# bearcove/loona

Measured on AMD Instinct MI355X. Metric: Huffman header-literal decode GiB/s (device-resident) at 1/2/4/8 MI355X, higher is better.
Workload: dtype u8

## Files before the change

### loona_amd/csrc/hpk_ctx.hip

```cpp
#include <stdio.h>
#include <string.h>
#include <sys/mman.h>

#include <initializer_list>

#include "hpk_device.h"

#define HPK_VERSION "hpk 0.39 gfx950 decode v39 (every batch: wave fills, each wave with its own LDS window and image, lookups in a 13-bit two-symbol table, longest-first queue, slot end offsets by DPP, nontemporal window loads stopping at the chunk's last byte, nontemporal write-back; chunks by guided self-scheduling from 4M literals, fixed 96-literal chunks below; fills and long-literal phase: body steps with no fit tests while >= 31 bits are left (29 with the 12-bit table), then the wave fills' tails as four masked lookups with no fit test per code (checked steps only for a 14..30-bit code or a cut code in the tail) and the other kernels' checked tails (the long phase's at its refill points); long literals one lane each streaming from HBM after the fills, dense ranges listed longest-first; literals of >= 8 KiB by a whole workgroup in speculative pieces; compacted-output form: wave fills packed per workgroup from an LDS cursor into a bound layout made from the input offsets, each lane storing its two literals in unaligned 16-byte pieces; small-call mode: a persistent kernel behind a host-mapped doorbell); encode v5 (byte-balanced workgroup ranges, start map and DPP segmented scan, run accumulator, LDS image, live chunks only)"

static thread_local std::string t_last_error;

int hpk_set_err(const char* what, hipError_t e) {
    char buf[256];
    snprintf(buf, sizeof buf, "%s: %s", what, hipGetErrorString(e));
    t_last_error = buf;
    return HPK_E_DEVICE;
}

int hpk_set_err_msg(const char* what, int code) {
    t_last_error = what;
    return code;
}


extern "C" const char* hpk_version(void) { return HPK_VERSION; }

extern "C" const char* hpk_last_error(const hpk_ctx*) { return t_last_error.c_str(); }

extern "C" hpk_ctx* hpk_ctx_create(int device) {
    const hpk_tables* t = hpk_get_tables();
    if (!t) { hpk_set_err_msg("code table build failed", HPK_E_INVAL); return nullptr; }
    int ndev = 0;
    hipError_t e = hipGetDeviceCount(&ndev);
    if (e != hipSuccess || ndev <= 0) { hpk_set_err("hipGetDeviceCount", e); return nullptr; }
    if (device < 0 || device >= ndev) { hpk_set_err_msg("device index out of range", HPK_E_INVAL); return nullptr; }
    hpk_ctx* c = new hpk_ctx();
    c->device = device;
    auto fail = [&](const char* what, hipError_t err) {
        hpk_set_err(what, err);
        hpk_ctx_destroy(c);
        return (hpk_ctx*)nullptr;
    };
    if ((e = hipSetDevice(device)) != hipSuccess) return fail("hipSetDevice", e);
    hipDeviceProp_t prop;
    if ((e = hipGetDeviceProperties(&prop, device)) != hipSuccess) return fail("hipGetDeviceProperties", e);
    if (strncmp(prop.gcnArchName, "gfx950", 6) != 0) {
        hpk_set_err_msg("libhpk kernels are built for gfx950 only", HPK_E_NODEVICE);
        delete c;
        return nullptr;
    }
    c->num_cu = prop.multiProcessorCount;
    if ((e = hipStreamCreateWithFlags(&c->own, hipStreamNonBlocking)) != hipSuccess) return fail("hipStreamCreate", e);
    c->stream = c->own;
    if ((e = hipMalloc(&c->d_lut2, sizeof(t->lut2))) != hipSuccess) return fail("hipMalloc lut2", e);
    if ((e = hipMemcpy(c->d_lut2, t->lut2, sizeof(t->lut2), hipMemcpyHostToDevice)) != hipSuccess)
        return fail("upload lut2", e);
    if ((e = hipMalloc(&c->d_lut3, sizeof(t->lut3))) != hipSuccess) return fail("hipMalloc lut3", e);
    if ((e = hipMemcpy(c->d_lut3, t->lut3, sizeof(t->lut3), hipMemcpyHostToDevice)) != hipSuccess)
        return fail("upload lut3", e);
    if ((e = hipMalloc(&c->d_lut13, sizeof(t->lut13))) != hipSuccess) return fail("hipMalloc lut13", e);
    if ((e = hipMemcpy(c->d_lut13, t->lut13, sizeof(t->lut13), hipMemcpyHostToDevice)) != hipSuccess)
        return fail("upload lut13", e);
    if ((e = hipMalloc(&c->d_lo, sizeof(t->lo))) != hipSuccess) return fail("hipMalloc lo", e);
    if ((e = hipMalloc(&c->d_codes, 2 * 257 * sizeof(uint32_t))) != hipSuccess) return fail("hipMalloc codes", e);
    uint32_t packed[2 * 257];
    for (int s = 0; s < 257; ++s) {
        packed[s] = t->code[s];
        packed[257 + s] = t->len[s];
    }
    if ((e = hipMemcpy(c->d_lo, t->lo, sizeof(t->lo), hipMemcpyHostToDevice)) != hipSuccess) return fail("upload lo", e);
    if ((e = hipMemcpy(c->d_codes, packed, sizeof(packed), hipMemcpyHostToDevice)) != hipSuccess) return fail("upload codes", e);
    if ((e = hipHostMalloc((void**)&c->h_err, 64, hipHostMallocMapped | hipHostMallocCoherent)) != hipSuccess)
        return fail("hipHostMalloc err flag", e);
    *c->h_err = 0;
    if ((e = hipHostGetDevicePointer((void**)&c->d_err, c->h_err, 0)) != hipSuccess) return fail("err flag pointer", e);
    return c;
}

static int grow(void** p, size_t* cap, size_t need) {
    if (need <= *cap) return HPK_E_OK;
    size_t n = need + need / 4 + 4096;
    (void)hipFree(*p);
    *p = nullptr;
    *cap = 0;
    HIP_TRY(hipMalloc(p, n));
    *cap = n;
    return HPK_E_OK;
}

static int slot_acquire(hpk_ctx* c, hpk_slot** slot) {
    hpk_slot* s = nullptr;
    bool any = false;
    for (hpk_slot& k : c->slots) {
        if (k.used && k.stream == c->stream) s = &k;
        any |= k.used;
    }
    if (!s) {
        if (any && !c->slot_events) {
            c->slot_events = true;
            HIP_TRY(hipStreamSynchronize(c->own));
            for (hpk_slot& k : c->slots)
                if (k.stream == c->own) k.ev_set = false;
        }
        int j = 0;
        while (j < hpk_ctx::kSlots && c->slots[j].used) ++j;
        if (j == hpk_ctx::kSlots) {
            j = c->slot_next;
            c->slot_next = (j + 1) % hpk_ctx::kSlots;
            if (c->slots[j].ev_set) HIP_TRY(hipEventSynchronize(c->slots[j].ev));
        }
        s = &c->slots[j];
        s->stream = c->stream;
    }
    if (c->slot_events && !s->ev) HIP_TRY(hipEventCreateWithFlags(&s->ev, hipEventDisableTiming));
    *slot = s;
    return HPK_E_OK;
}

struct slot_need {
    DevBuf* buf;
    size_t bytes;
};
static int slot_reserve(hpk_ctx* c, hpk_slot* s, std::initializer_list<slot_need> needs) {
    bool small = false;
    for (const slot_need& nd : needs) small |= nd.buf->cap < nd.bytes;
    if (small) {
        if (s->ev_set)
            HIP_TRY(hipEventSynchronize(s->ev));
        else if (s->used)
            HIP_TRY(hipStreamSynchronize(c->own));
        for (const slot_need& nd : needs)
            if (int rc = grow(&nd.buf->p, &nd.buf->cap, nd.bytes)) return rc;
    }
    s->used = true;
    return HPK_E_OK;
}

static int slot_commit(hpk_ctx* c, hpk_slot* s) {
    if (!c->slot_events && c->stream == c->own) return HPK_E_OK;
    if (!s->ev) HIP_TRY(hipEventCreateWithFlags(&s->ev, hipEventDisableTiming));
    HIP_TRY(hipEventRecord(s->ev, c->stream));
    s->ev_set = true;
    return HPK_E_OK;
}

extern "C" void hpk_ctx_destroy(hpk_ctx* c) {
    if (!c) return;
    (void)hipSetDevice(c->device);
    (void)hpk_persist_stop(c);
    if (c->sm_stream) (void)hipStreamDestroy(c->sm_stream);
    if (c->h_sm) (void)hipHostFree(c->h_sm);
    (void)hipFree(c->d_sm_dev);
    (void)hipStreamSynchronize(c->stream);
    (void)hipFree(c->d_lut2);
    (void)hipFree(c->d_lut3);
    (void)hipFree(c->d_lut13);
    (void)hipFree(c->d_lo);
    (void)hipFree(c->d_codes);
    (void)hipFree(c->d_in);
    (void)hipFree(c->d_out);
    (void)hipFree(c->d_meta);
    (void)hipFree(c->d_st);
    if (c->h_err) (void)hipHostFree(c->h_err);
    if (c->h_pin) (void)hipHostFree(c->h_pin);
    for (hpk_slot& s : c->slots) {
        if (s.ev_set) (void)hipEventSynchronize(s.ev);
        for (DevBuf* b : {&s.long_list, &s.cp_bound, &s.cp_tmp, &s.cp_cursor, &s.pk_scratch, &s.pk_bound, &s.pk_tmp})
            (void)hipFree(b->p);
        if (s.ev) (void)hipEventDestroy(s.ev);
    }
    for (int j = 0; j < hpk_ctx::kMaxChunks; ++j) {
        if (c->ev_in[j]) (void)hipEventDestroy(c->ev_in[j]);
        if (c->ev_run[j]) (void)hipEventDestroy(c->ev_run[j]);
        if (c->ev_out[j]) (void)hipEventDestroy(c->ev_out[j]);
    }
    if (c->h2d) (void)hipStreamDestroy(c->h2d);
    if (c->d2h) (void)hipStreamDestroy(c->d2h);
    if (c->own) (void)hipStreamDestroy(c->own);
    delete c;
}

extern "C" int hpk_ctx_set_stream(hpk_ctx* c, void* s) {
    if (!c) return HPK_E_INVAL;
    if (s == HPK_STREAM_LEGACY)
        c->stream = (hipStream_t)0;
    else
        c->stream = s ? (hipStream_t)s : c->own;
    return HPK_E_OK;
}

extern "C" int hpk_host_register(void* ptr, size_t bytes) {
    if (!ptr || !bytes) return hpk_set_err_msg("null range", HPK_E_INVAL);
    HIP_TRY(hipHostRegister(ptr, bytes, hipHostRegisterDefault));
    return HPK_E_OK;
}

extern "C" int hpk_host_unregister(void* ptr) {
    if (!ptr) return hpk_set_err_msg("null pointer", HPK_E_INVAL);
    HIP_TRY(hipHostUnregister(ptr));
    return HPK_E_OK;
}

int hpk_ctx_pinned(hpk_ctx* c, size_t bytes, void** p) {
    if (bytes > c->h_pin_cap) {
        HIP_TRY(hipSetDevice(c->device));
        HIP_TRY(hipStreamSynchronize(c->stream));
        if (c->d2h) HIP_TRY(hipStreamSynchronize(c->d2h));
        if (c->h_pin) (void)hipHostFree(c->h_pin);
        c->h_pin = nullptr;
        c->h_pin_cap = 0;
        const size_t cap = bytes + bytes / 4 + (1u << 20);
        HIP_TRY(hipHostMalloc(&c->h_pin, cap, hipHostMallocDefault));
        c->h_pin_cap = cap;
    }
    *p = c->h_pin;
    return HPK_E_OK;
}

extern "C" int hpk_ctx_set_decode_kernel(hpk_ctx* c, int kind) {
    if (!c || kind < HPK_DECODE_AUTO || kind > HPK_DECODE_WAVE) return hpk_set_err_msg("bad decode kernel", HPK_E_INVAL);
    c->decode_kernel = kind;
    return HPK_E_OK;
}

extern "C" void* hpk_ctx_stream(hpk_ctx* c) { return c ? (void*)c->stream : nullptr; }

extern "C" int hpk_ctx_set_small_mode(hpk_ctx* c, uint32_t max_literals, int workgroups, uint32_t idle_ms) {
    if (!c) return HPK_E_INVAL;
    HIP_TRY(hipSetDevice(c->device));
    if (max_literals == 0) {
        const int rc = hpk_persist_stop(c);
        c->sm_max = 0;
        return rc;
    }
    if (workgroups < 1 || workgroups > 16 || workgroups >= c->num_cu || idle_ms < 1 || idle_ms > 10000 ||
        max_literals > (uint32_t)workgroups * 256u * 64u)
        return hpk_set_err_msg("small mode: 1-16 workgroups, 1-10000 ms idle, at most 64 literals per lane", HPK_E_INVAL);
    if (!c->h_sm) {
        HIP_TRY(hipStreamCreateWithFlags(&c->sm_stream, hipStreamNonBlocking));
        HIP_TRY(hipHostMalloc(&c->h_sm, 256, hipHostMallocMapped | hipHostMallocCoherent));
        memset(c->h_sm, 0, 256);
        HIP_TRY(hipHostGetDevicePointer(&c->d_sm, c->h_sm, 0));
        HIP_TRY(hipMalloc(&c->d_sm_dev, 128));
    }
    if (c->sm_launched && (workgroups != c->sm_wgs || idle_ms != c->sm_idle_ms))
        if (int rc = hpk_persist_stop(c)) return rc;
    c->sm_max = max_literals;
    c->sm_wgs = workgroups;
    c->sm_idle_ms = idle_ms;
    return c->sm_launched ? HPK_E_OK : hpk_persist_start(c);
}

extern "C" int hpk_ctx_sync(hpk_ctx* c) {
    if (!c) return HPK_E_INVAL;
    HIP_TRY(hipStreamSynchronize(c->stream));
    return HPK_E_OK;
}

static int check_offsets(const uint32_t* off, uint32_t n, size_t cap) {
    for (uint32_t i = 0; i < n; ++i)
        if (off[i + 1] < off[i]) return hpk_set_err_msg("offsets must be non-decreasing", HPK_E_INVAL);
    if (off[n] > cap || off[n] > HPK_MAX_OFFSET) return hpk_set_err_msg("offsets pass the blob's capacity", HPK_E_INVAL);
    return HPK_E_OK;
}

static int take_err(hpk_ctx* c) {
    if (!__atomic_exchange_n(c->h_err, 0u, __ATOMIC_ACQ_REL)) return HPK_E_OK;
    return hpk_set_err_msg("a batch had non-monotone offsets or offsets past a blob's capacity (HPK_BAD_OFFSETS)",
                           HPK_E_INVAL);
}

extern "C" int hpk_ctx_check(hpk_ctx* c) {
    if (!c) return HPK_E_INVAL;
    HIP_TRY(hipStreamSynchronize(c->stream));
    return take_err(c);
}

static int call_end(hpk_ctx* c, int flags) {
    if (flags & HPK_ASYNC) return HPK_E_OK;
    HIP_TRY(hipStreamSynchronize(c->stream));
    return take_err(c);
}

typedef int (*launch_fn)(hpk_ctx*, const hpk_batch&);

static int decode_region(hpk_ctx* c, const hpk_batch& b) {
    hpk_slot* s;
    int rc;
    if ((rc = slot_acquire(c, &s)) || (rc = slot_reserve(c, s, {{&s->long_list, 4 * (size_t)b.n}}))) return rc;
    if ((rc = hpk_launch_decode(c, b, s->long_list.as<uint32_t>()))) return rc;
    return slot_commit(c, s);
}

static uint32_t clamp_cap(size_t cap) { return cap > HPK_MAX_OFFSET ? HPK_MAX_OFFSET : (uint32_t)cap; }

static int queue_chunks(launch_fn fn, hpk_ctx* c, const uint8_t* in_blob, const uint32_t* in_off, uint8_t* out_blob,
                        const uint32_t* out_off, uint32_t* out_len, uint8_t* status, uint32_t n, size_t in_bytes,
                        size_t out_bytes, int chunks, const uint32_t* cut, uint32_t* d_in_off, uint32_t* d_out_off,
                        uint32_t* d_len);

static int host_begin(launch_fn fn, hpk_ctx* c, const uint8_t* in_blob, size_t in_cap, const uint32_t* in_off,
                      uint32_t n, uint8_t* out_blob, size_t out_cap, const uint32_t* out_off, uint32_t* out_len,
                      uint8_t* status, bool trusted, int* nchunks, uint32_t* cut) {
    *nchunks = 0;
    if (!trusted && (check_offsets(in_off, n, in_cap) || check_offsets(out_off, n, out_cap))) return HPK_E_INVAL;
    if (n == 0) return HPK_E_OK;
    const size_t in_bytes = in_off[n], out_bytes = out_off[n];
    if ((in_bytes && !in_blob) || (out_bytes && !out_blob)) return hpk_set_err_msg("null blob", HPK_E_INVAL);
    int rc;
    if ((rc = grow((void**)&c->d_in, &c->d_in_cap, in_bytes + 16))) return rc;
    if ((rc = grow((void**)&c->d_out, &c->d_out_cap, out_bytes + 16))) return rc;
// ... 285 lines not shown
```

### loona_amd/csrc/hpk_wave.h

```cpp
#pragma once
#include <type_traits>

#include "hpk_decode_kernel.h"
#include "hpk_huge.h"
#include "hpk_long.h"

#ifndef HPK_BODY_UNROLL
#define HPK_BODY_UNROLL 4
#endif
#ifndef HPK_WAVE_TAB
#define HPK_WAVE_TAB 4
#endif
#ifndef HPK_CW_LANE_DIAG
#define HPK_CW_LANE_DIAG 0
#endif
#ifndef HPK_NT_STORE
#define HPK_NT_STORE 1
#endif
#ifndef HPK_NT_LOAD
#define HPK_NT_LOAD 1
#endif
#ifndef HPK_TAIL_MASKED
#define HPK_TAIL_MASKED 1
#endif
#ifndef HPK_WIN_CUT
#define HPK_WIN_CUT 1
#endif

namespace hpkdec {

typedef uint32_t v4u32 __attribute__((ext_vector_type(4)));
__device__ __forceinline__ void st16(uint4* p, const uint4 v) {
    if (HPK_NT_STORE) {
        const v4u32 x = {v.x, v.y, v.z, v.w};
        __builtin_nontemporal_store(x, reinterpret_cast<v4u32*>(p));
    } else {
        *p = v;
    }
}
__device__ __forceinline__ uint4 ld16(const uint4* p) {
    if (HPK_NT_LOAD) {
        const v4u32 x = __builtin_nontemporal_load(reinterpret_cast<const v4u32*>(p));
        return make_uint4(x.x, x.y, x.z, x.w);
    }
    return *p;
}

template <int kWinB, int kImgB, int kTab>
struct GeoW {
    static constexpr int kWaves = 16, kBlock = kWaves * 64;
    static constexpr int kWaveBytes = kWinB + kImgB;
    static constexpr int kLutBytes = 4 << lut_bits<kTab>();
    static constexpr int kLutOff = kLoBytes;
    static constexpr int kDummyOff = kLutOff + kLutBytes;
    static constexpr int kWaveOff = kDummyOff + 256;
    static constexpr int kCtrOff = kWaveOff + kWaves * kWaveBytes;
    static constexpr int kLdsBytes = kCtrOff + 64 + (int)kHugeMax * 4;
    static constexpr int kImg = kImgB;
    static_assert(kLoBytes % 16 == 0, "16-byte aligned carve-outs");
    static constexpr int kWinRounds = (kWinB / 16 + 63) / 64;
    static constexpr int kFlushRounds = (kImg / 16 + 1 + 63) / 64;
    static_assert(kLdsBytes <= 163840, "LDS budget (160 KiB per CU on gfx950)");
    static_assert(kWinB % 16 == 0 && kImgB % 16 == 0 && kWinB < 65536 && kImgB < 131072, "entry packing");
    static_assert(kWaves * kWaveBytes >= huge_lds_bytes<kBlock>(), "huge-phase LDS");
};

__device__ __forceinline__ uint32_t wave_incl_scan(uint32_t x, uint32_t lane) {
    x += (uint32_t)__builtin_amdgcn_update_dpp(0, (int)x, 0x111, 0xF, 0xF, false);
    x += (uint32_t)__builtin_amdgcn_update_dpp(0, (int)x, 0x112, 0xF, 0xF, false);
    x += (uint32_t)__builtin_amdgcn_update_dpp(0, (int)x, 0x114, 0xF, 0xF, false);
    x += (uint32_t)__builtin_amdgcn_update_dpp(0, (int)x, 0x118, 0xF, 0xF, false);
    const uint32_t r0 = (uint32_t)__builtin_amdgcn_readlane((int)x, 15);
    const uint32_t r1 = (uint32_t)__builtin_amdgcn_readlane((int)x, 31);
    const uint32_t r2 = (uint32_t)__builtin_amdgcn_readlane((int)x, 47);
    return x + (lane >= 16u ? r0 : 0u) + (lane >= 32u ? r1 : 0u) + (lane >= 48u ? r2 : 0u);
}

template <int kMode, int kWinB, int kImgB, uint32_t kChunk, int kGuided, int kRank, bool kCompact = false>
__global__ __launch_bounds__(1024) void hpk_decode_wave(DecodeArgs a) {
    constexpr int kTab = HPK_WAVE_TAB;
    using G = GeoW<kWinB, kMode == 3 ? kImgB - 64 : kImgB, kTab>;
    constexpr int kStore = kMode == 2 ? kNoStore : kPred;
    constexpr uint32_t kStamps = 13;
    __shared__ uint32_t s_dg[kMode == 3 ? G::kWaves * kStamps : 1];
    uint32_t tq = kMode == 3 ? (uint32_t)__builtin_amdgcn_s_memtime() : 0u;
    const uint32_t t_start = tq;
    auto dg_add = [&](int i, uint32_t v) {
        if (kMode == 3 && (threadIdx.x & 63u) == 0u) atomicAdd(&s_dg[(threadIdx.x >> 6) * kStamps + i], v);
    };
    auto stamp = [&](int i) {
        if (kMode == 3) {
            const uint32_t t = (uint32_t)__builtin_amdgcn_s_memtime();
            dg_add(i, t - tq);
            tq = t;
        }
    };
    constexpr int R = G::kWinRounds, F = G::kFlushRounds;
    __shared__ __attribute__((aligned(16))) uint8_t smem[G::kLdsBytes];
    uint16_t* s_lo = reinterpret_cast<uint16_t*>(smem);
    uint32_t* s_lut = reinterpret_cast<uint32_t*>(smem + G::kLutOff);
    uint32_t* s_ctr = reinterpret_cast<uint32_t*>(smem + G::kCtrOff);
    uint32_t* s_huge = s_ctr + 16;
    const uint32_t tid = threadIdx.x, lane = tid & 63u, wv = tid >> 6;
    const uint32_t BA = (uint32_t)((uint64_t)a.n * blockIdx.x / gridDim.x);
    const uint32_t BB = (uint32_t)((uint64_t)a.n * (blockIdx.x + 1) / gridDim.x);
    static_assert(G::kBlock == 1024, "the dense check's two offsets rounds");
    const uint32_t c0 = kGuided == 2 ? kChunk : max(kChunk, (BB - BA) / 32u);
    const uint32_t cur0 = kGuided == 0 ? BA + (uint32_t)((uint64_t)(BB - BA) * wv / G::kWaves) : min(BA + wv * c0, BB);
    const uint32_t ce0 =
        kGuided == 0 ? BA + (uint32_t)((uint64_t)(BB - BA) * (wv + 1) / G::kWaves) : min(cur0 + c0, BB);
    const uint32_t gin0 = a.in_off[cur0];
    const uint32_t gend0 = HPK_WIN_CUT ? a.in_off[ce0] : 0u;
    const uint32_t gout0 = kCompact ? 0u : a.out_off[cur0];
    const uint32_t kd = min(BB - BA, 2048u);
    uint32_t dv0[2], dv1[2];
#pragma unroll
    for (int r = 0; r < 2; ++r) {
        const uint32_t tt = BA + min(tid + (uint32_t)G::kBlock * r, kd ? kd - 1u : 0u);
        dv0[r] = a.in_off[tt];
        dv1[r] = a.in_off[tt + 1u];
    }
    for (uint32_t t = tid; t < kLoBytes / 16; t += G::kBlock)
        reinterpret_cast<uint4*>(s_lo)[t] = reinterpret_cast<const uint4*>(a.lo)[t];
    for (uint32_t t = tid; t < (uint32_t)G::kLutBytes / 16; t += G::kBlock)
        reinterpret_cast<uint4*>(s_lut)[t] = reinterpret_cast<const uint4*>(kTab == 4 ? a.lut13 : kTab == 3 ? a.lut3 : a.lut2)[t];
    if (tid < 16) s_ctr[tid] = tid == 7 && kGuided ? min(G::kWaves * c0, BB - BA) : 0u;
    if (kMode == 3)
        for (uint32_t t = tid; t < (uint32_t)G::kWaves * kStamps; t += G::kBlock) s_dg[t] = 0;
    const uint32_t in_end = min(a.in_off[a.n], a.in_cap) + a.in_mis;
    const uint32_t last16 = in_end ? (in_end - 1) >> 4 : 0;
    const uint32_t in0 = kCompact ? a.in_off[0] : 0u;
    auto ulay = [&](uint32_t i, uint32_t io) -> uint32_t {
        const uint32_t d = io - in0, q = __umulhi(d, 0xCCCCCCCDu) >> 2;
        return d + 3u * q + (((d - 5u * q) * 39u) >> 6) + 4u * i;
    };
    auto oof = [&](uint32_t i) -> uint32_t { return kCompact ? ulay(i, a.in_off[i]) : a.out_off[i]; };
    if (kCompact && blockIdx.x == 0 && tid == 0) a.co_off[a.n] = ulay(a.n, a.in_off[a.n]);
    const uint32_t wg0 = kCompact && BA < BB ? oof(BA) : 0u;
    auto leave = [&](uint32_t i, uint32_t nb) {
        if (kCompact) a.co_off[i] = wg0 + atomicAdd(&s_ctr[9], ((nb * 8u) / 5u + 3u) & ~3u);
        if (nb >= HPK_HUGE_MIN && nb < kHugeLimit) {
            const uint32_t h = atomicAdd(&s_ctr[8], 1u);
            if (h < kHugeMax) {
                s_huge[h] = i;
                return;
            }
        }
        if (nb >= a.long_big)
            a.long_list[BA + atomicAdd(&s_ctr[1], 1u)] = i;
        else
            a.long_list[BB - 1u - atomicAdd(&s_ctr[2], 1u)] = i;
    };
    __syncthreads();
    bool dense = false;
    {
        uint32_t dlb = 0, dtb = 0;
#pragma unroll
        for (int r = 0; r < 2; ++r) {
            if (tid + (uint32_t)G::kBlock * r < kd) {
                const uint32_t nb = min(dv1[r] - dv0[r], 1u << 20);
                dtb += nb;
                dlb += nb >= a.long_min ? nb : 0u;
            }
        }
#pragma unroll
        for (int d = 32; d >= 1; d >>= 1) {
            dlb += __shfl_xor(dlb, d);
            dtb += __shfl_xor(dtb, d);
        }
        if (lane == 0 && dtb) {
            atomicAdd(&s_ctr[4], dlb);
            atomicAdd(&s_ctr[5], dtb);
        }
        __syncthreads();
        if (s_ctr[4] > s_ctr[5] / 2u) {
            uint32_t* const s_cls = reinterpret_cast<uint32_t*>(smem + G::kWaveOff);
            if (tid < 64) s_cls[tid] = 0;
            __syncthreads();
            bool no = false;
            for (uint32_t i = BA + tid; i < BB; i += G::kBlock) {
                const uint32_t p0 = a.in_off[i], p1 = a.in_off[i + 1];
                const uint32_t q0 = kCompact ? ulay(i, p0) : a.out_off[i], q1 = kCompact ? ulay(i + 1u, p1) : a.out_off[i + 1];
                const bool ok = p0 <= p1 && p1 <= a.in_cap && q0 <= q1 && q1 <= a.out_cap &&
                                (uint64_t)(q1 - q0) >= (uint64_t)(p1 - p0) * 8u / 5u;
                if (!ok) {
                    no = true;
                    continue;
                }
                const uint32_t nb = p1 - p0;
                if (!(nb >= HPK_HUGE_MIN && nb < kHugeLimit)) atomicAdd(&s_cls[lpt_class_of(nb)], 1u);
            }
            if (__any(no) && lane == 0) s_ctr[6] = 1u;
            __syncthreads();
            dense = s_ctr[6] == 0u;
            if (dense) {
                if (tid < 64) {
                    const uint32_t v = tid < 32 ? s_cls[tid] : 0u;
                    uint32_t x = v;
#pragma unroll
                    for (int d = 1; d < 64; d <<= 1) {
                        const uint32_t y = __shfl_up(x, d);
                        if (lane >= (uint32_t)d) x += y;
                    }
                    if (tid < 32) s_cls[32 + tid] = x - v;
                    if (tid == 31) s_ctr[1] = x;
                }
                __syncthreads();
                for (uint32_t i = BA + tid; i < BB; i += G::kBlock) {
                    const uint32_t nb = a.in_off[i + 1] - a.in_off[i];
                    if (kCompact) a.co_off[i] = wg0 + atomicAdd(&s_ctr[9], ((nb * 8u) / 5u + 3u) & ~3u);
                    bool huge = false;
                    if (nb >= HPK_HUGE_MIN && nb < kHugeLimit) {
                        const uint32_t hh = atomicAdd(&s_ctr[8], 1u);
                        if (hh < kHugeMax) {
                            s_huge[hh] = i;
                            huge = true;
                        }
                    }
                    if (!huge)
                        a.long_list[nb >= HPK_HUGE_MIN && nb < kHugeLimit ? BB - 1u - atomicAdd(&s_ctr[2], 1u)
                                                                          : BA + atomicAdd(&s_cls[32 + lpt_class_of(nb)], 1u)] = i;
                }
                __syncthreads();
            }
            if (!dense) {
                __syncthreads();
                if (tid == 0) {
                    s_ctr[1] = 0;
                    s_ctr[2] = 0;
                    s_ctr[8] = 0;
                    s_ctr[9] = 0;
                }
                __syncthreads();
            }
        }
    }
    if (!dense) {
        uint8_t* const s_win = smem + G::kWaveOff + wv * G::kWaveBytes;
        uint8_t* const s_img = s_win + kWinB;
        const uint32_t* const win32 = reinterpret_cast<const uint32_t*>(s_win);
        const uint32_t wbits = (uint32_t)(G::kWaveOff + wv * G::kWaveBytes) * 8u;
        const uint32_t obase = (uint32_t)(G::kWaveOff + wv * G::kWaveBytes + kWinB);
        const uint32_t* const wl32 = reinterpret_cast<const uint32_t*>(smem);
        uint8_t* const ol8 = smem;
        const uint32_t dmy = (uint32_t)G::kDummyOff + lane * 4u;
        bool given = false;
        auto claim = [&](uint32_t& ca, uint32_t& ce) {
            if (!kGuided) {
                ca = given ? BB : BA + (uint32_t)((uint64_t)(BB - BA) * wv / G::kWaves);
                ce = given ? BB : BA + (uint32_t)((uint64_t)(BB - BA) * (wv + 1) / G::kWaves);
                given = true;
                return;
            }
            uint32_t c = 0;
            if (lane == 0) {
                const uint32_t seen = *(volatile HPK_LDS_AS uint32_t*)(&s_ctr[7]);
                const uint32_t left = BB - BA > seen ? BB - BA - seen : 0u;
                const uint32_t want = kGuided == 2 ? kChunk : max(kChunk, left / 32u);
                c = atomicAdd(&s_ctr[7], want);
                c = c < BB - BA ? c : BB - BA;
                ce = BA + min(c + want, BB - BA);
            }
            ca = BA + (uint32_t)__builtin_amdgcn_readfirstlane((int)c);
            ce = (uint32_t)__builtin_amdgcn_readfirstlane((int)ce);
        };
        uint32_t io0[2], oo0[2], ie = 0, oe = 0, pcnt = 1, pc = 0;
        uint4 ch[R];
        constexpr bool kCut = HPK_WIN_CUT != 0;
        constexpr uint32_t kWinC = (uint32_t)kWinB / 16u;
        auto chunk_lim = [&](uint32_t x) {
            x = min(x, a.in_cap) + a.in_mis;
            return min(last16, x ? (x - 1u) >> 4 : 0u);
        };
        uint32_t clim = kCut ? chunk_lim(gend0) : last16;
        auto prefetch = [&](uint32_t c, uint32_t e, uint32_t base16) {
            const uint32_t cnt = min(128u, e - c);
#pragma unroll
            for (int r = 0; r < 2; ++r) {
                const uint32_t t = c + min(lane + 64u * r, cnt - 1u);
                io0[r] = a.in_off[t];
                if (!kCompact) oo0[r] = a.out_off[t];
            }
            ie = a.in_off[c + cnt];
            if (!kCompact) oe = a.out_off[c + cnt];
            pcnt = cnt;
            pc = c;
            const uint4* g16 = reinterpret_cast<const uint4*>(a.in_base);
#pragma unroll
            for (int r = 0; r < R; ++r) ch[r] = ld16(g16 + min((base16 >> 4) + lane + 64u * r, clim));
        };
        uint32_t io1[2], oo1[2];
        auto ends = [&]() {
            if (kCompact) {
#pragma unroll
                for (int r = 0; r < 2; ++r) oo0[r] = ulay(pc + min(lane + 64u * r, pcnt - 1u), io0[r]);
                oe = ulay(pc + pcnt, ie);
            }
            const uint32_t i1 = (uint32_t)__builtin_amdgcn_readfirstlane((int)io0[1]);
            const uint32_t o1 = (uint32_t)__builtin_amdgcn_readfirstlane((int)oo0[1]);
#pragma unroll
            for (int r = 0; r < 2; ++r) {
                const uint32_t ni = (uint32_t)__builtin_amdgcn_update_dpp((int)(r ? ie : i1), (int)io0[r], 0x130, 0xF, 0xF, false);
                const uint32_t no = (uint32_t)__builtin_amdgcn_update_dpp((int)(r ? oe : o1), (int)oo0[r], 0x130, 0xF, 0xF, false);
                const bool last = lane + 64u * r + 1u >= pcnt;
                io1[r] = last ? ie : ni;
                oo1[r] = last ? oe : no;
            }
        };
        uint32_t cur = cur0, ce = ce0;
        given = true;
        uint32_t gin = 0, gout = 0;
        uint32_t sens[4] = {0u, 1u, 2u, 3u};
        if (cur < ce) {
            gin = gin0 + a.in_mis;
            gout = (kCompact ? ulay(cur, gin0) : gout0) + a.out_mis;
            prefetch(cur, ce, gin & ~15u);
        }
        uint32_t pk = 0, pcur = 0, pG0 = 0, pG1 = 0;
        uint32_t rv0 = 0, rv1 = 0, ri0 = 0xFFFFFFFFu, ri1 = 0xFFFFFFFFu;
        uint32_t stop = 0;
        stamp(11);
        auto opaque = [](uint32_t x) {
            asm volatile("" : "+v"(x));
            return x;
        };
        auto flush = [&]() {
            const uint32_t ob = pG0 & ~15u;
            const uint32_t c0 = ob >> 4, c1 = (pG1 + 15u) >> 4;
            uint4* l16 = reinterpret_cast<uint4*>(s_img) + (opaque(lane) - lane);
            uint4* g16 = reinterpret_cast<uint4*>(a.out_base);
            if (kMode != 2) {
                if (lane < 32) {
                    const uint32_t g = lane < 16 ? c0 << 4 : (c1 - 1u) << 4;
                    const bool partial = !(g >= pG0 && g + 16u <= pG1) && (lane < 16 || c1 - 1u != c0);
                    const uint32_t x = g + (lane & 15u);
                    if (partial && x >= pG0 && x < pG1) a.out_base[x] = s_img[x - ob];
                }
#pragma unroll
                for (int r = 0; r < F; ++r) {
                    const uint32_t ci = c0 + lane + 64u * r;
                    if (ci < c1) {
                        if ((ci << 4) >= pG0 && (ci << 4) + 16u <= pG1) st16(g16 + ci, l16[ci - c0]);
                    }
                }
            }
            if (ri0 != 0xFFFFFFFFu) {
                a.out_len[pcur + ri0] = rv0 & 0xFFFFFFu;
                a.status[pcur + ri0] = (uint8_t)(rv0 >> 24);
            }
            if (ri1 != 0xFFFFFFFFu) {
                a.out_len[pcur + ri1] = rv1 & 0xFFFFFFu;
                a.status[pcur + ri1] = (uint8_t)(rv1 >> 24);
            }
            ri0 = ri1 = 0xFFFFFFFFu;
        };
        auto compact_fill = [&](uint32_t fcur, uint32_t fk, const uint2 q1, const uint2 q2) {
            uint32_t* const s_len = reinterpret_cast<uint32_t*>(s_win);
            uint32_t* const s_ex = s_len + 128;
            static_assert(256 * 4 <= kWinB, "compact tables in the window");
            s_len[lane] = kListed;
            s_len[lane + 64u] = kListed;
            if (ri0 != 0xFFFFFFFFu) s_len[ri0] = rv0;
            if (ri1 != 0xFFFFFFFFu) s_len[ri1] = rv1;
            const uint32_t l0 = s_len[lane], l1 = s_len[lane + 64u];
            const uint32_t x0 = l0 == kListed ? 0u : l0 & 0xFFFFFFu, x1 = l1 == kListed ? 0u : l1 & 0xFFFFFFu;
            const uint32_t i0 = wave_incl_scan(x0, lane), i1 = wave_incl_scan(x1, lane);
            const uint32_t t0 = (uint32_t)__builtin_amdgcn_readlane((int)i0, 63);
            const uint32_t ex0 = i0 - x0, ex1 = t0 + i1 - x1;
            const uint32_t tot = t0 + (uint32_t)__builtin_amdgcn_readlane((int)i1, 63);
            uint32_t u = 0;
            if (lane == 0) u = atomicAdd(&s_ctr[9], tot);
            const uint32_t base = wg0 + (uint32_t)__builtin_amdgcn_readfirstlane((int)u);
            if (tot != 0u) {
                const uint32_t D0 = a.out_mis + base;
                s_ex[lane] = ex0;
                s_ex[lane + 64u] = ex1;
                __builtin_amdgcn_wave_barrier();
                const uint32_t* const img32 = reinterpret_cast<const uint32_t*>(s_img);
                uint32_t js[2], jd[2], jn[2];
#pragma unroll
                for (int r = 0; r < 2; ++r) {
                    const uint32_t ri = r ? ri1 : ri0, rv = r ? rv1 : rv0;
                    const bool on = ri != 0xFFFFFFFFu && rv != kListed;
                    js[r] = ((r ? q2.y : q1.y) >> 12) & 0x1FFFFu;
                    jd[r] = D0 + s_ex[on ? ri : 0u];
                    jn[r] = on ? rv & 0xFFFFFFu : 0u;
                }
                auto dw_at = [&](uint32_t u) {
                    return __builtin_amdgcn_alignbyte(img32[(u >> 2) + 1u], img32[u >> 2], u & 3u);
                };
                uint32_t sp = js[0], dp = jd[0], np = jn[0], tp = 0;
                bool second = true;
                if (np == 0u) {
                    sp = js[1];
                    dp = jd[1];
                    np = jn[1];
                    second = false;
                }
                while (HPK_CW_LANE_DIAG != 2 && __any(tp < np)) {
                    if (tp < np) {
                        if (np >= 16u) {
                            const uint32_t t = min(tp, np - 16u), u = sp + t;
                            const uint32_t sw = u >> 2, s3 = u & 3u;
                            uint32_t A[5];
#pragma unroll
                            for (int j = 0; j < 5; ++j) A[j] = img32[sw + (uint32_t)j];
                            u32x4u v;
                            v.x = __builtin_amdgcn_alignbyte(A[1], A[0], s3);
                            v.y = __builtin_amdgcn_alignbyte(A[2], A[1], s3);
                            v.z = __builtin_amdgcn_alignbyte(A[3], A[2], s3);
                            v.w = __builtin_amdgcn_alignbyte(A[4], A[3], s3);
                            if (HPK_CW_LANE_DIAG == 3)
                                *reinterpret_cast<u32x4u*>(a.out_base + ((dp + t) & ~15u)) = v;
                            else if (HPK_CW_LANE_DIAG == 4)
                                asm volatile("" ::"v"(v.x), "v"(v.y), "v"(v.z), "v"(v.w));
                            else
                                *reinterpret_cast<u32x4u*>(a.out_base + dp + t) = v;
                            tp += 16u;
                        } else if (np >= 4u) {
                            u32u* const g = reinterpret_cast<u32u*>(a.out_base + dp);
                            g[0] = dw_at(sp);
                            if (np >= 8u) g[1] = dw_at(sp + 4u);
                            if (np >= 12u) g[2] = dw_at(sp + 8u);
                            *reinterpret_cast<u32u*>(a.out_base + dp + np - 4u) = dw_at(sp + np - 4u);
                            tp = np;
                        } else {
                            for (uint32_t b = 0; b < np; ++b) a.out_base[dp + b] = s_img[sp + b];
                            tp = np;
                        }
                        if (tp >= np && second) {
                            sp = js[1];
                            dp = jd[1];
                            np = jn[1];
                            tp = 0;
                            second = false;
                        }
                    }
                }
            }
            if (lane < fk && l0 != kListed) {
                a.co_off[fcur + lane] = base + ex0;
                a.out_len[fcur + lane] = x0;
                a.status[fcur + lane] = (uint8_t)(l0 >> 24);
            }
            if (lane + 64u < fk && l1 != kListed) {
                a.co_off[fcur + lane + 64u] = base + ex1;
                a.out_len[fcur + lane + 64u] = x1;
                a.status[fcur + lane + 64u] = (uint8_t)(l1 >> 24);
            }
        };
        while (cur < ce) {
            const uint32_t cntl = min(128u, ce - cur);
            const uint32_t base16 = gin & ~15u, ob16 = gout & ~15u;
            bool bad = false;
            uint32_t ex[2], ey[2];
            bool fits[2];
            ends();
#pragma unroll
            for (int r = 0; r < 2; ++r) {
                const uint32_t t = lane + 64u * r;
                bad |= t < cntl && !(io0[r] <= io1[r] && io1[r] <= a.in_cap && oo0[r] <= oo1[r] && oo1[r] <= a.out_cap);
                const uint32_t p0 = io0[r] + a.in_mis, p1 = io1[r] + a.in_mis;
                const uint32_t o0 = oo0[r] + a.out_mis, o1 = oo1[r] + a.out_mis;
                fits[r] = t < cntl && p1 - base16 <= (uint32_t)kWinB && o1 - ob16 <= (uint32_t)G::kImg;
                const uint32_t nbytes = p1 - p0, ocap = o1 - o0;
                const bool fast = ocap >= (nbytes * 8u) / 5u;
                ex[r] = (p0 - base16) | (nbytes << 16);
                ey[r] = t | ((o0 - ob16) << 12) | (fast ? 0u : kQ7Byte);
            }
            const bool wbad = __any(bad) || stop != 0u;
            stamp(1);
            dg_add(8, 1u);
            if (wbad) {
                if (pk) flush();
                pk = 0;
                if (lane == 0) {
                    *a.err = 1u;
                    s_ctr[0] = 1u;
                }
                for (;;) {
                    for (uint32_t i = cur + lane; i < ce; i += 64u) {
                        a.out_len[i] = 0;
                        a.status[i] = (uint8_t)HPK_BAD_OFFSETS;
                    }
                    claim(cur, ce);
                    if (cur >= ce) break;
                }
                break;
            }
            const uint64_t f0 = __ballot(fits[0]), f1 = __ballot(fits[1]);
            const uint32_t k = (uint32_t)__popcll(f0) + (uint32_t)__popcll(f1);
            if (k == 0) {
                if (pk) flush();
                pk = 0;
                const uint32_t nb = a.in_off[cur + 1] - a.in_off[cur];
                const bool left = nb >= a.long_min && oof(cur + 1) - oof(cur) >= (nb * 8u) / 5u;
                if (lane == 0) {
                    if (left) {
                        leave(cur, nb);
                    } else {
                        const GlobalSrc g{reinterpret_cast<const uint32_t*>(a.in_base), last16 * 4 + 3};
                        uint8_t* dst = a.out_base + gout;
                        if (kCompact) {
                            const uint32_t o = wg0 + atomicAdd(&s_ctr[9], ((nb * 8u) / 5u + 3u) & ~3u);
                            a.co_off[cur] = o;
                            dst = a.out_base + a.out_mis + o;
                        }
                        Lit L = {};
                        lit_bytes_to(L, g, s_lo, [&](uint32_t j, uint8_t v) { dst[j] = v; },
                                     oof(cur + 1) - oof(cur), gin, a.in_off[cur + 1] + a.in_mis - gin);
                        a.out_len[cur] = L.cnt;
                        a.status[cur] = (uint8_t)lit_status(L);
                    }
                }
                cur += 1;
                if (cur == ce) {
                    claim(cur, ce);
                    if (kCut && cur < ce) clim = chunk_lim(a.in_off[ce]);
                }
                if (cur < ce) {
                    gin = a.in_off[cur] + a.in_mis;
                    gout = oof(cur) + a.out_mis;
                    prefetch(cur, ce, gin & ~15u);
                }
                continue;
            }
            const uint64_t fl = f1 ? f1 : f0;
            const int hl = 63 - __builtin_clzll(fl);
            const uint32_t gin_end = (uint32_t)__builtin_amdgcn_readlane((int)((f1 ? io1[1] : io1[0]) + a.in_mis), hl);
            const uint32_t gout_end =
                (uint32_t)__builtin_amdgcn_readlane((int)((f1 ? oo1[1] : oo1[0]) + a.out_mis), hl);
            uint32_t cur_n = cur + k, ce_n = ce, gin_n = gin_end, gout_n = gout_end;
            if (cur_n == ce) {
                claim(cur_n, ce_n);
                if (cur_n < ce_n) {
                    gin_n = a.in_off[cur_n] + a.in_mis;
                    gout_n = oof(cur_n) + a.out_mis;
                    if (kCut) clim = chunk_lim(a.in_off[ce_n]);
                }
            }
            {
                uint4* l16 = reinterpret_cast<uint4*>(s_win) + (opaque(lane) - lane);
#pragma unroll
                for (int r = 0; r < R; ++r) {
                    const uint4 c = ch[r];
                    const uint32_t j = lane + 64u * r;
                    if (j < kWinC)
                        l16[j] = make_uint4(__builtin_bswap32(c.x), __builtin_bswap32(c.y), __builtin_bswap32(c.z),
                                            __builtin_bswap32(c.w));
                }
            }
            stamp(4);
            if (pk) flush();
            stamp(2);
            bool qd[2];
            uint32_t key[2];
#pragma unroll
            for (int r = 0; r < 2; ++r) {
                const uint32_t nbytes = ex[r] >> 16;
                const bool lng = nbytes >= a.long_min && !(ey[r] & kQ7Byte);
                if (fits[r] && lng) leave(cur + lane + 64u * r, nbytes);
                qd[r] = fits[r] && !lng;
                key[r] = kRank == 1 ? min(nbytes >> 2, 15u) : min(nbytes >> 1, 31u);
            }
            uint32_t rank0 = 0, rank1 = 0, kq = 0;
            uint2* const q = reinterpret_cast<uint2*>(s_img + 256);
            if (kRank == 0) {
                uint32_t* const hist = reinterpret_cast<uint32_t*>(s_img);
                if (lane < 32) hist[lane] = 0;
                const uint32_t pa = qd[0] ? atomicAdd(&hist[31u - key[0]], 1u) : 0u;
                const uint32_t pb = qd[1] ? atomicAdd(&hist[31u - key[1]], 1u) : 0u;
                const uint32_t v = lane < 32 ? hist[lane] : 0u;
                uint32_t x = v;
                x += (uint32_t)__builtin_amdgcn_update_dpp(0, (int)x, 0x111, 0xF, 0xF, false);
                x += (uint32_t)__builtin_amdgcn_update_dpp(0, (int)x, 0x112, 0xF, 0xF, false);
                x += (uint32_t)__builtin_amdgcn_update_dpp(0, (int)x, 0x114, 0xF, 0xF, false);
                x += (uint32_t)__builtin_amdgcn_update_dpp(0, (int)x, 0x118, 0xF, 0xF, false);
                const uint32_t row0 = (uint32_t)__builtin_amdgcn_readlane((int)x, 15);
                x += lane >= 16u ? row0 : 0u;
                if (lane < 32) hist[32 + lane] = x - v;
                kq = (uint32_t)__builtin_amdgcn_readlane((int)x, 31);
                rank0 = qd[0] ? hist[32 + 31 - key[0]] + pa : 0u;
                rank1 = qd[1] ? hist[32 + 31 - key[1]] + pb : 0u;
            }
#pragma unroll
            for (int c = (kRank == 1 ? 15 : 31); kRank != 0 && c >= 0; --c) {
                const bool h0 = qd[0] && key[0] == (uint32_t)c, h1 = qd[1] && key[1] == (uint32_t)c;
                const uint64_t m0 = __ballot(h0), m1 = __ballot(h1);
                const uint32_t p0 = (uint32_t)__popcll(m0);
                const uint32_t b0 = __builtin_amdgcn_mbcnt_hi((uint32_t)(m0 >> 32), __builtin_amdgcn_mbcnt_lo((uint32_t)m0, 0u));
                const uint32_t b1 = __builtin_amdgcn_mbcnt_hi((uint32_t)(m1 >> 32), __builtin_amdgcn_mbcnt_lo((uint32_t)m1, 0u));
                rank0 = h0 ? kq + b0 : rank0;
                rank1 = h1 ? kq + p0 + b1 : rank1;
                kq += p0 + (uint32_t)__popcll(m1);
            }
            if (qd[0]) q[rank0] = make_uint2(ex[0], ey[0]);
            if (qd[1]) q[rank1] = make_uint2(ex[1], ey[1]);
            stamp(3);
            const uint32_t t1 = lane, t2 = 127u - lane;
            const uint2 e1 = kq ? q[min(t1, kq - 1u)] : make_uint2(0u, 0u);
            const uint2 e2 = kq ? q[min(t2, kq - 1u)] : make_uint2(0u, 0u);
            stop = *(volatile HPK_LDS_AS uint32_t*)(&s_ctr[0]);
            {
                const bool more = cur_n < ce_n;
                prefetch(more ? cur_n : cur, more ? ce_n : cur + k, (more ? gin_n : gin) & ~15u);
            }
            Lit12 L, N;
            auto load = [&](Lit12& T, const uint2 e, uint32_t tt) {
                T.act = tt < kq && !(e.y & kQ7Byte);
                T.idx = e.y & 0xFFFu;
                const uint32_t nb = e.x >> 16;
                const uint32_t o = (e.y >> 12) & 0x1FFFFu;
                T.X = wbits + (e.x & 0xFFFFu) * 8u + 31u;
                T.Eb = T.X + (T.act ? nb * 8u : 0u);
                T.o = obase + o;
                T.o0 = obase + o;
                T.st = HPK_OK;
                T.prog = false;
                lit12_load(T, wl32);
            };
            load(L, e1, t1);
            uint32_t sX = 0, sO = 0, sSt = 0;
            bool s1 = false;
            stamp(5);
            uint32_t Lend = 0;
            if (kMode != 1) {
                bool body = L.Eb - L.X >= body_min<kTab>();
                uint32_t aX = L.X, aO = L.o, aSt = L.st;
                bool aAct = L.act, onA = true;
                for (;;) {
                    dg_add(9, 1u);
#pragma unroll
                    for (int s = 0; s < HPK_BODY_UNROLL; ++s) {
                        if (body)
                            lit12_body<kStore, kTab, (kMode >= 8 && kMode <= 10) ? kMode - 7 : 0>(L, wl32, s_lut, s_lo, ol8,
                                                                                                   body);
                        if (kMode == 6) {
#pragma unroll
                            for (int q = 0; q < 4; ++q) {
                                asm volatile("v_xor_b32 %0, %0, %1" : "+v"(sens[0]) : "v"(L.X));
                                asm volatile("v_xor_b32 %0, %0, %1" : "+v"(sens[1]) : "v"(L.o));
                                asm volatile("v_xor_b32 %0, %0, %1" : "+v"(sens[2]) : "v"(L.Eb));
                                asm volatile("v_xor_b32 %0, %0, %1" : "+v"(sens[3]) : "v"(L.d1));
                            }
                        }
                    }
                    if (__any(!body)) {
                        const bool sw = !body & onA;
                        if (sw) {
                            aX = L.X;
                            aO = L.o;
                            aSt = L.st;
                            aAct = L.act;
                            load(L, e2, t2);
                            onA = false;
                            body = L.Eb - L.X >= body_min<kTab>();
                        }
                        if (!__any(body)) break;
                    }
                }
                N = L;
                L.X = aX;
                L.o = aO;
                L.st = aSt;
                L.act = aAct;
                L.Eb = wbits + (e1.x & 0xFFFFu) * 8u + 31u + (aAct ? (e1.x >> 16) * 8u : 0u);
                L.o0 = obase + ((e1.y >> 12) & 0x1FFFFu);
                L.idx = e1.y & 0xFFFu;
                if (aSt != HPK_OK) L.Eb = L.X;
                lit12_load(L, wl32);
                L.more = L.Eb - L.X >= 5u;
                N.more = N.Eb - N.X >= 5u;
                stamp(12);
                if (HPK_TAIL_MASKED) {
                    Tail12 TL, TN;
                    tail12_begin(TL, L);
                    tail12_begin(TN, N);
#pragma unroll
                    for (int s = 0; s < 4; ++s) {
                        tail12_look<kStore, kTab>(TL, s_lut, ol8, dmy);
                        tail12_look<kStore, kTab>(TN, s_lut, ol8, dmy);
                    }
                    L.more &= tail12_end<kTab>(TL, L);
                    N.more &= tail12_end<kTab>(TN, N);
                }
                while (__any(L.more | N.more)) {
                    if (L.more) lit12_step<kStore, true, kTab, true>(L, wl32, s_lut, s_lo, ol8, dmy);
                    if (N.more) lit12_step<kStore, true, kTab, true>(N, wl32, s_lut, s_lo, ol8, dmy);
                }
                sX = L.X;
                sO = L.o;
                sSt = L.st;
                s1 = L.act;
                L = N;
                Lend = L.o;
            }
            stamp(6);
            if (kMode == 6 && (sens[0] ^ sens[1] ^ sens[2] ^ sens[3]) == 0x5EB51u)
                a.status[0] = 9u;
            {
                const uint32_t Eb = wbits + (e1.x & 0xFFFFu) * 8u + 31u + (e1.x >> 16) * 8u;
                const uint32_t st = sSt != HPK_OK ? sSt : residual_status(Eb - sX, win_at(wl32, sX - 31u));
                rv0 = (sO - obase - ((e1.y >> 12) & 0x1FFFFu)) | (st << 24);
                ri0 = s1 ? e1.y & 0xFFFu : 0xFFFFFFFFu;
                rv1 = (Lend - L.o0) | (lit12_status(L) << 24);
                ri1 = L.act ? L.idx : 0xFFFFFFFFu;
            }
            if (kMode == 1) {
                rv0 = 0;
                ri0 = t1 < kq ? e1.y & 0xFFFu : 0xFFFFFFFFu;
            }
#pragma unroll
            for (int r = 0; r < 2; ++r) {
                const uint2 e = r == 0 ? e1 : e2;
                const uint32_t tt = r == 0 ? t1 : t2;
                if (tt < kq && (e.y & kQ7Byte)) {
                    const uint32_t i = e.y & 0xFFFu;
                    const uint32_t o = (e.y >> 12) & 0x1FFFFu;
                    Lit B = {};
                    lit_bytes_to(B, LdsSwapSrc{win32}, s_lo, [&](uint32_t j, uint8_t v) { s_img[o + j] = v; },
                                 oof(cur + i + 1) - oof(cur + i), e.x & 0xFFFFu, e.x >> 16);
                    if (r == 0) {
                        rv0 = B.cnt | (lit_status(B) << 24);
                        ri0 = i;
                    } else {
                        rv1 = B.cnt | (lit_status(B) << 24);
                        ri1 = i;
                    }
                }
            }
            stamp(7);
            if (kCompact) {
#pragma unroll
                for (int r = 0; r < 2; ++r) asm volatile("" ::"v"(io0[r]), "s"(ie));
#pragma unroll
                for (int r = 0; r < R; ++r) asm volatile("" ::"v"(ch[r].x), "v"(ch[r].y), "v"(ch[r].z), "v"(ch[r].w));
                compact_fill(cur, k, e1, e2);
            } else {
                pk = k;
                pcur = cur;
                pG0 = gout;
                pG1 = gout_end;
            }
            cur = cur_n;
            ce = ce_n;
            gin = gin_n;
            gout = gout_n;
        }
        if (pk) flush();
        stamp(2);
    }
    __syncthreads();
    const uint32_t c1 = s_ctr[1], c2 = s_ctr[2], nh = min(s_ctr[8], kHugeMax);
    huge_phase<G::kBlock, kTab>(a, s_huge, nh, reinterpret_cast<uint32_t*>(smem + G::kWaveOff), s_lut, s_lo);
    if (c1 + c2) {
        static_assert(G::kWaveOff % 16 == 0, "long-phase rings");
        uint8_t* const area = smem + G::kWaveOff;
        constexpr int kLB = HPK_LONG_WAVES * 64;
        constexpr int kLQ = kLB * (HPK_LONG_RING * 4 + HPK_LONG_OS);
        static_assert(kLQ + HPK_LONG_WAVES * HPK_LONG_CLAIM * 16 <= G::kWaves * G::kWaveBytes, "long-phase LDS");
        long_phase<kLB, HPK_LONG_U, HPK_LONG_RING, kMode == 5 ? 1 : 0, G::kBlock, HPK_LONG_OS, HPK_LONG_CLAIM, kTab>(
            a, BA, BB, c1, c2, &s_ctr[3], reinterpret_cast<uint32_t*>(area), area + kLB * HPK_LONG_RING * 4,
            reinterpret_cast<uint4*>(area + kLQ), s_lut, s_lo);
    }
    stamp(10);
    if (kMode == 3) {
        __syncthreads();
        if (lane < kStamps) {
            const uint32_t v = lane == 0 ? (uint32_t)__builtin_amdgcn_s_memtime() - t_start : s_dg[wv * kStamps + lane];
            a.dbg[((uint64_t)blockIdx.x * G::kWaves + wv) * 16u + lane] = v;
        }
    }
}

}
```

Before: 1211.

## Split write-back into LDS read and deferred stores; issue next prefetch before stores

The previous image's write-back is split into two steps. The LDS read-out happens right after the window is staged, and the global stores are deferred until after the longest-first sort and queue build, so the sort overlaps the LDS read latency. The next fill's window prefetch is now issued before the write-back stores, so its loads are in flight while stores drain. In exchange the wave holds F extra uint4 registers, the sort reuses the image region (checked by a static_assert), and rank computation is now unconditional.

```diff
diff --git a/loona_amd/csrc/hpk_ctx.hip b/loona_amd/csrc/hpk_ctx.hip
--- a/loona_amd/csrc/hpk_ctx.hip
+++ b/loona_amd/csrc/hpk_ctx.hip
@@ -6,7 +6,7 @@
 
 #include "hpk_device.h"
 
-#define HPK_VERSION "hpk 0.39 gfx950 decode v39 (every batch: wave fills, each wave with its own LDS window and image, lookups in a 13-bit two-symbol table, longest-first queue, slot end offsets by DPP, nontemporal window loads stopping at the chunk's last byte, nontemporal write-back; chunks by guided self-scheduling from 4M literals, fixed 96-literal chunks below; fills and long-literal phase: body steps with no fit tests while >= 31 bits are left (29 with the 12-bit table), then the wave fills' tails as four masked lookups with no fit test per code (checked steps only for a 14..30-bit code or a cut code in the tail) and the other kernels' checked tails (the long phase's at its refill points); long literals one lane each streaming from HBM after the fills, dense ranges listed longest-first; literals of >= 8 KiB by a whole workgroup in speculative pieces; compacted-output form: wave fills packed per workgroup from an LDS cursor into a bound layout made from the input offsets, each lane storing its two literals in unaligned 16-byte pieces; small-call mode: a persistent kernel behind a host-mapped doorbell); encode v5 (byte-balanced workgroup ranges, start map and DPP segmented scan, run accumulator, LDS image, live chunks only)"
+#define HPK_VERSION "hpk 0.40 gfx950 decode v40 (every batch: wave fills, each wave with its own LDS window and image, lookups in a 13-bit two-symbol table, longest-first queue sorted under the previous image's LDS read-out, the next fill's loads issued ahead of the write-back's stores, slot end offsets by DPP, nontemporal window loads stopping at the chunk's last byte, nontemporal write-back; chunks by guided self-scheduling from 4M literals, fixed 96-literal chunks below; fills and long-literal phase: body steps with no fit tests while >= 31 bits are left (29 with the 12-bit table), then the wave fills' tails as four masked lookups with no fit test per code (checked steps only for a 14..30-bit code or a cut code in the tail) and the other kernels' checked tails (the long phase's at its refill points); long literals one lane each streaming from HBM after the fills, dense ranges listed longest-first; literals of >= 8 KiB by a whole workgroup in speculative pieces; compacted-output form: wave fills packed per workgroup from an LDS cursor into a bound layout made from the input offsets, each lane storing its two literals in unaligned 16-byte pieces; small-call mode: a persistent kernel behind a host-mapped doorbell); encode v5 (byte-balanced workgroup ranges, start map and DPP segmented scan, run accumulator, LDS image, live chunks only)"
 
 static thread_local std::string t_last_error;
 
diff --git a/loona_amd/csrc/hpk_wave.h b/loona_amd/csrc/hpk_wave.h
--- a/loona_amd/csrc/hpk_wave.h
+++ b/loona_amd/csrc/hpk_wave.h
@@ -22,6 +22,12 @@
 #endif
 #ifndef HPK_TAIL_MASKED
 #define HPK_TAIL_MASKED 1
+#endif
+#ifndef HPK_FLUSH_SPLIT
+#define HPK_FLUSH_SPLIT 1
+#endif
+#ifndef HPK_PF_EARLY
+#define HPK_PF_EARLY 1
 #endif
 #ifndef HPK_WIN_CUT
 #define HPK_WIN_CUT 1
@@ -324,6 +330,7 @@
             asm volatile("" : "+v"(x));
             return x;
         };
+        auto sgpr = [](uint32_t x) { return (uint32_t)__builtin_amdgcn_readfirstlane((int)x); };
         auto flush = [&]() {
             const uint32_t ob = pG0 & ~15u;
             const uint32_t c0 = ob >> 4, c1 = (pG1 + 15u) >> 4;
@@ -343,6 +350,48 @@
                         if ((ci << 4) >= pG0 && (ci << 4) + 16u <= pG1) st16(g16 + ci, l16[ci - c0]);
                     }
                 }
+            }
+            if (ri0 != 0xFFFFFFFFu) {
+                a.out_len[pcur + ri0] = rv0 & 0xFFFFFFu;
+                a.status[pcur + ri0] = (uint8_t)(rv0 >> 24);
+            }
+            if (ri1 != 0xFFFFFFFFu) {
+                a.out_len[pcur + ri1] = rv1 & 0xFFFFFFu;
+                a.status[pcur + ri1] = (uint8_t)(rv1 >> 24);
+            }
+            ri0 = ri1 = 0xFFFFFFFFu;
+        };
+        uint4 fl[F];
+        uint32_t fpb = 0;
+        constexpr uint32_t kImgC = (uint32_t)G::kImg / 16u;
+        auto flush_read = [&]() {
+            const uint32_t ob = sgpr(pG0) & ~15u;
+            const uint32_t c0 = ob >> 4, c1 = (sgpr(pG1) + 15u) >> 4;
+            const uint4* l16 = reinterpret_cast<const uint4*>(s_img) + (opaque(lane) - lane);
+            const uint32_t x = ((lane & 16u) ? (c1 - 1u) << 4 : c0 << 4) + (lane & 15u);
+            fpb = s_img[min(x - ob, (uint32_t)G::kImg - 1u)];
+#pragma unroll
+            for (int r = 0; r < F; ++r) fl[r] = l16[min(lane + 64u * r, kImgC - 1u)];
+        };
+        auto flush_store = [&]() {
+            const uint32_t g0 = sgpr(pG0), g1 = sgpr(pG1);
+            const uint32_t ob = g0 & ~15u;
+            const uint32_t c0 = ob >> 4, c1 = (g1 + 15u) >> 4;
+            uint4* g16 = reinterpret_cast<uint4*>(a.out_base);
+            if (kMode != 2) {
+                if (lane < 32) {
+                    const uint32_t g = lane < 16 ? c0 << 4 : (c1 - 1u) << 4;
+                    const bool partial = !(g >= g0 && g + 16u <= g1) && (lane < 16 || c1 - 1u != c0);
+                    const uint32_t x = g + (lane & 15u);
+                    if (partial && x >= g0 && x < g1) a.out_base[x] = (uint8_t)fpb;
+                }
+                const uint32_t lo = (g0 + 15u) >> 4, hi = g1 >> 4;
+                const uint32_t cnt = hi > lo ? hi - lo : 0u;
+                const uint32_t t = lane - (lo - c0);
+                uint4* const p = g16 + c0 + opaque(lane);
+#pragma unroll
+                for (int r = 0; r < F; ++r)
+                    if (t + 64u * r < cnt) st16(p + 64 * r, fl[r]);
             }
             if (ri0 != 0xFFFFFFFFu) {
                 a.out_len[pcur + ri0] = rv0 & 0xFFFFFFu;
@@ -539,7 +588,7 @@
                     if (kCut) clim = chunk_lim(a.in_off[ce_n]);
                 }
             }
-            {
+            auto stage = [&]() {
                 uint4* l16 = reinterpret_cast<uint4*>(s_win) + (opaque(lane) - lane);
 #pragma unroll
                 for (int r = 0; r < R; ++r) {
@@ -549,10 +598,15 @@
                         l16[j] = make_uint4(__builtin_bswap32(c.x), __builtin_bswap32(c.y), __builtin_bswap32(c.z),
                                             __builtin_bswap32(c.w));
                 }
-            }
+            };
+            constexpr bool kSplit = HPK_FLUSH_SPLIT != 0 && !kCompact, kPfEarly = HPK_PF_EARLY != 0;
+            stage();
             stamp(4);
-            if (pk) flush();
+            if (!kSplit && pk) flush();
+            if (kSplit) flush_read();
+            asm volatile("" ::: "memory");
             stamp(2);
+            static_assert(256 + 128 * 8 <= G::kImg, "the sort's counts and queue in the image");
             bool qd[2];
             uint32_t key[2];
 #pragma unroll
@@ -580,8 +634,8 @@
                 x += lane >= 16u ? row0 : 0u;
                 if (lane < 32) hist[32 + lane] = x - v;
                 kq = (uint32_t)__builtin_amdgcn_readlane((int)x, 31);
-                rank0 = qd[0] ? hist[32 + 31 - key[0]] + pa : 0u;
-                rank1 = qd[1] ? hist[32 + 31 - key[1]] + pb : 0u;
+                rank0 = hist[32 + 31 - key[0]] + pa;
+                rank1 = hist[32 + 31 - key[1]] + pb;
             }
 #pragma unroll
             for (int c = (kRank == 1 ? 15 : 31); kRank != 0 && c >= 0; --c) {
@@ -596,15 +650,20 @@
             }
             if (qd[0]) q[rank0] = make_uint2(ex[0], ey[0]);
             if (qd[1]) q[rank1] = make_uint2(ex[1], ey[1]);
-            stamp(3);
             const uint32_t t1 = lane, t2 = 127u - lane;
             const uint2 e1 = kq ? q[min(t1, kq - 1u)] : make_uint2(0u, 0u);
             const uint2 e2 = kq ? q[min(t2, kq - 1u)] : make_uint2(0u, 0u);
             stop = *(volatile HPK_LDS_AS uint32_t*)(&s_ctr[0]);
-            {
+            stamp(3);
+            auto prefetch_next = [&]() {
                 const bool more = cur_n < ce_n;
                 prefetch(more ? cur_n : cur, more ? ce_n : cur + k, (more ? gin_n : gin) & ~15u);
-            }
+            };
+            if (kPfEarly) prefetch_next();
+            stamp(5);
+            if (kSplit && pk) flush_store();
+            stamp(2);
+            if (!kPfEarly) prefetch_next();
             Lit12 L, N;
             auto load = [&](Lit12& T, const uint2 e, uint32_t tt) {
                 T.act = tt < kq && !(e.y & kQ7Byte);
```

After: 1230 (median of 6 runs). 1.6% higher.
